# YichengDWu/tinyedm

Measured on AMD Instinct MI355X. Metric: train imgs/sec CIFAR-10 32x32 bf16, higher is better.
Workload: dtype bf16; 1 GPU; CIFAR-10 32x32 unconditional EDM2 U-Net (conf/cifar10.yaml, 35.6M params) full training step: diffuse+embed+denoiser fwd/bwd+loss+grad all-reduce+Adam+EMA; per_gpu_batch=128, global_batch=128, parallelism=dp1, conditional=False, step_launch=hipGraph replay, collective=none

## Files before the change

include/tinyedm_hip.h:

```cpp
#ifndef TINYEDM_HIP_H
#define TINYEDM_HIP_H
#ifdef __cplusplus
extern "C" {
#endif

typedef struct ihipStream_t* edm_stream_t;

int edm_version(void);
const char* edm_last_error(void);
int edm_init(int device);
int edm_graph_replay_safe(void);
typedef struct {
  unsigned step, seed_lo, seed_hi, reserved;
  float lr, ema_beta, grad_scale, bc1, bc2sqrt, pad[3];
} edm_step_params;

int edm_conv_igemm(const void* X, const void* Wp, void* Y, const void* R, float alpha, float beta, int B, int H,
                   int W, int Cin, int Cout, int taps, edm_stream_t stream);
int edm_conv_igemm_v2(const void* X, const void* Wp, void* Y, const void* R, float alpha, float beta, int B, int H,
                      int W, int Cin, int Cout, int taps, edm_stream_t stream);
int edm_conv_igemm_v6(const void* X, const void* Wp, void* Y, const void* R, float alpha, float beta, int B, int H,
                      int W, int Cin, int Cout, int taps, edm_stream_t stream);
int edm_conv_igemm_s(const void* X, const void* Wp, void* Y, const void* R, float alpha, float beta, int B, int H,
                     int W, int Cin, int Cout, int taps, edm_stream_t stream);
// ... 82 lines not shown
int edm_attention_fwd(const void* qkv, void* y, int B, int N, int C, int heads, edm_stream_t stream);
int edm_attention_bwd(const void* qkv, const void* y, const void* gy, void* gqkv, int B, int N, int C, int heads,
                      edm_stream_t stream);

int edm_attention_long_supported(int N, int C, int heads);
int edm_attention_long_fwd(const void* qkv, void* y, float* stat, int B, int N, int C, int heads, edm_stream_t stream);
int edm_attention_long_bwd(const void* qkv, const void* y, const void* gy, const float* stat, void* gqkv, float* work,
                           int B, int N, int C, int heads, edm_stream_t stream);

int edm_attention_qkv_supported(int N, int C, int heads);
int edm_attention_qkv_fwd(const void* x, const void* Wqkv, void* y, void* stat, int B, int N, int C, int heads,
                          int heads_per_wg, edm_stream_t stream);
int edm_attention_qkv_bwd(const void* x, const void* y, const void* gout, const void* stat, const void* Wqkv,
                          const void* Wd_out, void* gqkv, float alpha, int B, int N, int C, int heads, int heads_per_wg,
                          edm_stream_t stream);

int edm_pixelnorm_silu_fwd(const void* x, void* xn, void* a, float* dsave, long P, int C, edm_stream_t stream);
int edm_pixelnorm_silu_bwd(const void* xn, const float* dsave, const void* gxn, float gxn_scale, const void* ga,
                           const void* gadd, void* gx, long P, int C, edm_stream_t stream);
int edm_pool_pixelnorm_silu_fwd(const void* x, void* xn, void* a, float* dsave, int B, int Hp, int Wp, int C,
                                edm_stream_t stream);
int edm_pool_pixelnorm_silu_bwd(const void* xn, const float* dsave, const void* gxn, float gxn_scale, const void* ga,
                                const void* gadd, void* gx, int B, int Hp, int Wp, int C, edm_stream_t stream);
int edm_silu_fwd(const void* x, void* a, long n, edm_stream_t stream);
int edm_silu_bwd(const void* x, const void* ga, const void* gextra, float extra_scale, void* gx, long n,
                 edm_stream_t stream);
int edm_axpby(const void* a, float alpha, const void* b, float beta, void* out, long n, edm_stream_t stream);
int edm_mod_silu_drop_fwd(const void* r, const float* lin, long lin_stride, const float* gain, void* a, int B, int HW,
                          int C, float pdrop, unsigned long long seed, unsigned sub, unsigned step, const void* dyn,
                          edm_stream_t stream);
int edm_mod_silu_drop_bwd(const void* r, const float* lin, long lin_stride, const float* gain, const void* ga, void* gr,
                          float* gm, float* glin, long glin_stride, float* ggain, int B, int HW, int C, float pdrop,
                          unsigned long long seed, unsigned sub, unsigned step, const void* dyn, edm_stream_t stream);
int edm_mod_silu_drop_bwd_raw(const void* r, const float* lin, long lin_stride, const float* gain, const void* ga, void* gr,
                              float* gm, long gm_stride, int B, int HW, int C, float pdrop, unsigned long long seed,
                              unsigned sub, unsigned step, const void* dyn, edm_stream_t stream);
int edm_dropout_mask(unsigned char* mask, long n, float pdrop, unsigned long long seed, unsigned sub, unsigned step,
                     edm_stream_t stream);
int edm_pool2(const void* x, void* y, int B, int Hout, int Wout, int C, float scale, edm_stream_t stream);
int edm_up2(const void* x, const void* add, void* y, int B, int Hout, int Wout, int C, float scale, edm_stream_t stream);
int edm_up2_silu(const void* x, void* y, void* a, int B, int Hout, int Wout, int C, edm_stream_t stream);
int edm_reduce_hw(const void* x, long x_stride, const void* y, long y_stride, float* out, int B, int HW, int C,
                  float scale, edm_stream_t stream);
int edm_scalelong_fwd(const float* mean, const float* W1h, const float* W2h, float* gate, float* z1save, int B, int C,
                      int R, edm_stream_t stream);
int edm_scalelong_bwd(const float* mean, const float* W1h, const float* W2h, const float* gate, const float* z1save,
// ... 278 lines not shown
```

tinyedm_amd/_lib.py:

```python
import ctypes
import os

_HERE = os.path.dirname(os.path.abspath(__file__))
LIB_PATH = os.environ.get("EDM_LIB_PATH") or os.path.join(_HERE, "libtinyedm_hip.so")

P, I, L, F = ctypes.c_void_p, ctypes.c_int, ctypes.c_long, ctypes.c_float
U, U64 = ctypes.c_uint, ctypes.c_ulonglong
D = ctypes.c_double

SIGNATURES = {
    "edm_version": [],
    "edm_last_error": [],
    "edm_init": [I],
    "edm_graph_replay_safe": [],
    "edm_pixelnorm_silu_fwd": [P, P, P, P, L, I, P],
    "edm_pixelnorm_silu_bwd": [P, P, P, F, P, P, P, L, I, P],
    "edm_pool_pixelnorm_silu_fwd": [P, P, P, P, I, I, I, I, P],
    "edm_pool_pixelnorm_silu_bwd": [P, P, P, F, P, P, P, I, I, I, I, P],
    "edm_up2_silu": [P, P, P, I, I, I, I, P],
    "edm_silu_fwd": [P, P, L, P],
    "edm_silu_bwd": [P, P, P, F, P, L, P],
    "edm_axpby": [P, F, P, F, P, L, P],
    "edm_mod_silu_drop_fwd": [P, P, L, P, P, I, I, I, F, U64, U, U, P, P],
    "edm_mod_silu_drop_bwd": [P, P, L, P, P, P, P, P, L, P, I, I, I, F, U64, U, U, P, P],
    "edm_mod_silu_drop_bwd_raw": [P, P, L, P, P, P, P, L, I, I, I, F, U64, U, U, P, P],
    "edm_dropout_mask": [P, L, F, U64, U, U, P],
    "edm_pool2": [P, P, I, I, I, I, F, P],
    "edm_up2": [P, P, P, I, I, I, I, F, P],
    "edm_reduce_hw": [P, L, P, L, P, I, I, I, F, P],
    "edm_scalelong_fwd": [P, P, P, P, P, I, I, I, P],
    "edm_scalelong_bwd": [P, P, P, P, P, P, P, P, P, I, I, I, P],
    "edm_skip_gate_fwd": [P, P, P, P, P, P, I, I, I, I, P],
    "edm_skip_gate_bwd": [P, L, I, P, P, P, P, P, P, P, P, P, P, I, I, I, I, P],
    "edm_skip_gate_wgrad_multi": [P, I, P, P, I, P],
    "edm_skip_gate_wgrad_multi_table_bytes": [],
    "edm_skip_gate_fwd_multi": [P, I, P, P, I, P],
    "edm_skip_gate_fwd_multi_table_bytes": [],
    "edm_skip_gate_bwd_multi": [P, I, P, P, I, P],
    "edm_skip_half_bwd_multi": [P, I, P, P, I, P],
    "edm_skip_gate_bwd_multi_table_bytes": [],
    "edm_concat_gate_fwd": [P, P, P, P, P, I, I, I, I, P],
# ... 243 lines not shown
```

tinyedm_amd/csrc/elementwise.hip:

```cpp
#include "common.h"
#include <stdarg.h>
#include <stdio.h>

static thread_local char g_err[512] = "";
extern "C" void edm_set_error(const char* fmt, ...) {
  va_list ap;
  va_start(ap, fmt);
  vsnprintf(g_err, sizeof(g_err), fmt, ap);
  va_end(ap);
}
extern "C" const char* edm_last_error() { return g_err; }
extern "C" int edm_version() { return 1; }

static inline int cdiv(long a, long b) { return (int)((a + b - 1) / b); }
static inline int grid_for(long work, int block, int cap = 256 * 16) {
  long g = (work + block - 1) / block;
  if (g > cap) g = cap;
  if (g < 1) g = 1;
  return (int)g;
}

template <int LPP, bool POOL = false>
__global__ __launch_bounds__(256) void k_pnorm_silu_fwd(const bf16* __restrict__ x, bf16* __restrict__ xn,
                                                          bf16* __restrict__ a, float* __restrict__ dsave, int P,
// ... 35 lines not shown
      }
    }
    ss = group_sum<LPP>(ss);
    const float d = NORM_EPS + sqrtf(ss) * rsC;
    const float inv = 1.0f / d;
#pragma unroll
    for (int it = 0; it < 2; ++it) {
      const int c8 = lig + it * LPP;
      if (pv && c8 < CL) {
        float o[8], s[8];
#pragma unroll
        for (int i = 0; i < 8; ++i) {
          o[i] = (float)(bf16)(v[it][i] * inv);
          s[i] = mp_silu_b(o[i]);
        }
        store8(xn + p * C + c8 * 8, o);
        store8(a + p * C + c8 * 8, s);
      }
    }
    if (pv && lig == 0) dsave[p] = d;
  }
}

template <int LPP, bool UP = false>
__global__ __launch_bounds__(256) void k_pnorm_silu_bwd(const bf16* __restrict__ xn, const float* __restrict__ dsave,
                                                          const bf16* __restrict__ gxn, float gs,
                                                          const bf16* __restrict__ ga, const bf16* __restrict__ gadd,
                                                          bf16* __restrict__ gx, int P, int C, int Hp = 0, int Wp = 0) {
  constexpr int GPW = 64 / LPP;
  const int lane = threadIdx.x & 63, wave = threadIdx.x >> 6;
  const int lig = lane % LPP, grp = lane / LPP;
  const int CL = C >> 3;
  const long stride = (long)gridDim.x * 4 * GPW;
  for (long p0 = ((long)blockIdx.x * 4 + wave) * GPW; p0 < P; p0 += stride) {
    const long p = p0 + grp;
    const bool pv = p < P;
    float y[2][8], g[2][8];
    float dot = 0.f;
#pragma unroll
    for (int it = 0; it < 2; ++it) {
      const int c8 = lig + it * LPP;
      if (pv && c8 < CL) {
        load8(xn + p * C + c8 * 8, y[it]);
        float t[8];
        if (gxn) {
          load8(gxn + p * C + c8 * 8, t);
#pragma unroll
          for (int i = 0; i < 8; ++i) g[it][i] = gs * t[i];
        } else {
#pragma unroll
          for (int i = 0; i < 8; ++i) g[it][i] = 0.f;
// ... 14 lines not shown
    float inv = 1.0f / d;
#pragma unroll
    for (int it = 0; it < 2; ++it) {
      const int c8 = lig + it * LPP;
      if (pv && c8 < CL) {
        float o[8];
#pragma unroll
        for (int i = 0; i < 8; ++i) o[i] = (g[it][i] - y[it][i] * coef) * inv;
        if constexpr (UP) {
          const int w = (int)(p % Wp);
          const long t2 = p / Wp;
          const int h = (int)(t2 % Hp);
          const long b = t2 / Hp;
          const long e0 = ((b * 2 * Hp + 2 * h) * 2 * Wp + 2 * w) * C + c8 * 8;
          const long row = (long)2 * Wp * C;
#pragma unroll
          for (int i = 0; i < 8; ++i) o[i] = 0.25f * (float)(bf16)o[i];
#pragma unroll
          for (int q = 0; q < 4; ++q) {
            const long e = e0 + (q >> 1) * row + (q & 1) * C;
            float r[8];
#pragma unroll
            for (int i = 0; i < 8; ++i) r[i] = o[i];
            if (gadd) {
              float t[8];
              load8(gadd + e, t);
#pragma unroll
              for (int i = 0; i < 8; ++i) r[i] += t[i];
            }
            store8(gx + e, r);
          }
          continue;
        }
        if (gadd) {
          float t[8];
          load8(gadd + p * C + c8 * 8, t);
#pragma unroll
          for (int i = 0; i < 8; ++i) o[i] += t[i];
        }
        store8(gx + p * C + c8 * 8, o);
      }
    }
  }
}

static int pick_lpp(int C) {
  int cl = C / 8;
  return cl <= 16 ? 16 : (cl <= 32 ? 32 : 64);
}

extern "C" int edm_pixelnorm_silu_fwd(const void* x, void* xn, void* a, float* dsave, long P, int C,
                                      hipStream_t st) {
  EDM_REQUIRE(P > 0 && P < (1L << 31) && C > 0 && C % 8 == 0 && C <= 1024, "pixelnorm_silu_fwd: bad P=%ld C=%d", P, C);
  int lpp = pick_lpp(C);
  int gpw = 64 / lpp;
  int grid = grid_for(P, 4 * gpw);
#define L(N) hipLaunchKernelGGL(k_pnorm_silu_fwd<N>, dim3(grid), dim3(256), 0, st, (const bf16*)x, (bf16*)xn, (bf16*)a, dsave, (int)P, C)
// ... 23 lines not shown
  EDM_REQUIRE(xn && dsave && gx && B > 0 && Hp > 0 && Wp > 0 && C > 0 && C % 8 == 0 && C <= 1024 &&
                  (long)B * Hp * Wp < (1L << 31), "pool_pixelnorm_silu_bwd: bad args");
  const long P = (long)B * Hp * Wp;
  int lpp = pick_lpp(C);
  int gpw = 64 / lpp;
  int grid = grid_for(P, 4 * gpw);
#define L(N) hipLaunchKernelGGL((k_pnorm_silu_bwd<N, true>), dim3(grid), dim3(256), 0, st, (const bf16*)xn, dsave, (const bf16*)gxn, gxn_scale, (const bf16*)ga, (const bf16*)gadd, (bf16*)gx, (int)P, C, Hp, Wp)
  if (lpp == 16) L(16); else if (lpp == 32) L(32); else L(64);
#undef L
  EDM_CHECK_LAUNCH("pool_pixelnorm_silu_bwd");
  return EDM_OK;
}

extern "C" int edm_pixelnorm_silu_bwd(const void* xn, const float* dsave, const void* gxn, float gxn_scale,
                                      const void* ga, const void* gadd, void* gx, long P, int C, hipStream_t st) {
  EDM_REQUIRE(P > 0 && P < (1L << 31) && C > 0 && C % 8 == 0 && C <= 1024, "pixelnorm_silu_bwd: bad P=%ld C=%d", P, C);
  int lpp = pick_lpp(C);
  int gpw = 64 / lpp;
  int grid = grid_for(P, 4 * gpw);
#define L(N) hipLaunchKernelGGL(k_pnorm_silu_bwd<N>, dim3(grid), dim3(256), 0, st, (const bf16*)xn, dsave, (const bf16*)gxn, gxn_scale, (const bf16*)ga, (const bf16*)gadd, (bf16*)gx, (int)P, C)
  if (lpp == 16) L(16); else if (lpp == 32) L(32); else L(64);
#undef L
  EDM_CHECK_LAUNCH("pixelnorm_silu_bwd");
  return EDM_OK;
}

__global__ void k_silu_fwd(const bf16* __restrict__ x, bf16* __restrict__ a, long n8) {
  for (long i = (long)blockIdx.x * blockDim.x + threadIdx.x; i < n8; i += (long)gridDim.x * blockDim.x) {
    float v[8];
    load8(x + i * 8, v);
#pragma unroll
    for (int j = 0; j < 8; ++j) v[j] = mp_silu_b(v[j]);
    store8(a + i * 8, v);
  }
}
__global__ void k_silu_bwd(const bf16* __restrict__ x, const bf16* __restrict__ ga, const bf16* __restrict__ ge,
                           float s, bf16* __restrict__ gx, long n8) {
  for (long i = (long)blockIdx.x * blockDim.x + threadIdx.x; i < n8; i += (long)gridDim.x * blockDim.x) {
    float v[8], g[8], e[8];
    load8(x + i * 8, v);
    load8(ga + i * 8, g);
    if (ge) load8(ge + i * 8, e);
#pragma unroll
    for (int j = 0; j < 8; ++j) g[j] = mp_silu_grad_b(v[j]) * g[j] + (ge ? s * e[j] : 0.f);
    store8(gx + i * 8, g);
  }
// ... 1358 lines not shown
```

tinyedm_amd/networks.py:

```python
from __future__ import annotations

import contextlib
import math
import os
from typing import Optional

import numpy as np
import torch
import torch.nn as nn
from torch import Tensor

from . import ops

bf16, f32 = torch.bfloat16, torch.float32


class _Rng:
    seed: int = 42
    step: int = 0
    dyn = None


rng = _Rng()

# ... 82 lines not shown
                _flush_fin(key)
            _queue_backward_end(w.device)
            return None
        g = ops.wgrad_finish(slabs, w.data, self._taps(), I, perm=self._perm, scale=scale)
        return g.view_as(w)


WGRAD_STREAM = os.environ.get("EDM_WGRAD_STREAM", "1") != "0"
W3_GROUP = max(0, min(ops.W3_MAX_LAYERS, int(os.environ.get("EDM_W3_GROUP", "16"))))
W3_TAIL = max(0, int(os.environ.get("EDM_W3_TAIL", "0")))
_w3_seen = {}
_w3_total = {}
W3_MAXPIX = int(os.environ.get("EDM_W3_MAXPIX", str(1 << 18)))
FIN_GROUP = 40
W1_GROUP = max(0, min(16, int(os.environ.get("EDM_W1_GROUP", "16"))))
_w1_pending = {}
_bwd_end_queued = set()
MOD_DEFER_UNFUSED = os.environ.get("EDM_MOD_DEFER_UNFUSED", "1") != "0"
SG_MULTI = os.environ.get("EDM_SG_MULTI", "1") != "0"
SG_HALVES = os.environ.get("EDM_SG_HALVES", "1") != "0"
SG_BWD_MULTI = os.environ.get("EDM_SG_BWD_MULTI", "1") != "0"
SG_DEFER = os.environ.get("EDM_SG_DEFER", "1") != "0"
_sg_pending = {}
_w3_pending = {}
TAIL_LOWRANK = os.environ.get("EDM_TAIL_LOWRANK", "1") != "0"
_tail_slot = {}
TAIL_FWD = os.environ.get("EDM_TAIL_FWD", "1") != "0"
_tail_fwd_slot = {}
_fin_pending = {}


def _run_on_side(device, fn, tensors=()):
    if WGRAD_STREAM:
        side = ops.side_stream(device)
        side.wait_stream(torch.cuda.current_stream())
        with torch.cuda.stream(side):
            fn()
        for t in tensors:
            t.record_stream(side)
    else:
        fn()


class FusedOptPass:

    def __init__(self, base, ema, dyn):
# ... 64 lines not shown
    _run_on_side(dev, lambda: ops.wgrad_finish_multi(args), [a[0] for a in args])
    for _, w, *_rest in items:
        w._edm_deferred = False
        for hook in getattr(w, "_edm_hooks", ()):
            hook(w)


def _flush_sg(key):
    items = _sg_pending.pop(key, None)
    if not items:
        return
    outs = ops.skip_gate_wgrad_multi([(ws, mean, R) for _, ws, mean, R in items])
    for (sl, _, _, _), (gw1h, gw2h) in zip(items, outs):
        sl.layer1.finish_grad(gw1h.view(1, 1, *gw1h.shape))
        sl.layer2.finish_grad(gw2h.view(1, 1, *gw2h.shape))


def _backward_end(key):
    _bwd_end_queued.discard(key)
    _tail_slot.pop(key, None)
    _tail_fwd_slot.pop(key, None)
    if key in _w3_seen:
        _w3_total[key] = _w3_seen.pop(key)
    _flush_sg(key)
    _flush_w3(key)
    _flush_fin(key)
    if WGRAD_STREAM:
        torch.cuda.current_stream(key).wait_stream(ops.side_stream(key))


def _queue_backward_end(device):
    key = torch.device(device).index
    if key in _bwd_end_queued:
        return
    try:
        torch.autograd.Variable._execution_engine.queue_callback(lambda: _backward_end(key))
        _bwd_end_queued.add(key)
    except RuntimeError:
        _backward_end(key)


def reset_backward_state():
    _tail_slot.clear()
    _tail_fwd_slot.clear()
    if _bwd_end_queued or _w3_pending or _fin_pending or _w1_pending or _sg_pending:
        _bwd_end_queued.clear()
        for items in _sg_pending.values():
            for sl, *_rest in items:
                sl.layer1.weight._edm_deferred = sl.layer2.weight._edm_deferred = False
        _sg_pending.clear()
        for items in _w1_pending.values():
            for m, _, _, _ in items:
                m.weight._edm_deferred = False
        _w1_pending.clear()
        for items in _fin_pending.values():
            for _, w, *_rest in items:
                w._edm_deferred = False
        _fin_pending.clear()
        for items in _w3_pending.values():
            for m, _, _, _ in items:
                m.weight._edm_deferred = False
        _w3_pending.clear()
        _w3_seen.clear()
        if WGRAD_STREAM:
            for s in ops.side_streams():
                torch.cuda.current_stream(s.device).wait_stream(s)

# ... 611 lines not shown
        gw_qkv = _wgrad(mod.qkv_conv, x, gqkv, 1)
        return gx, gw_qkv, gw_out, None, None, None


class _ResBlockFn(torch.autograd.Function):

    @staticmethod
    def forward(ctx, u, emb, w1x1, w1, w2, wemb, gain, blk, lin_view, glin_view, token, s_pre=None, alias=False,
                gm_view=None, skip=None, w_sl1=None, w_sl2=None, pre=None, dest=None, pool=False, gate_pre=None, tail=0):
        enc = blk.is_encoder
        ctx.set_materialize_grads(False)
        has1 = w1x1 is not None
        taps = 9
        wf1, wd1, _ = blk.conv_3x3_1.packs()
        wf2, wd2, _ = blk.conv_3x3_2.packs()
        batched = lin_view is not None
        weh = None if batched else blk.embed.packs()[2]
        wf11 = wd11 = None
        tail_fwd = False
        ctx.has_skip = skip is not None
        if skip is not None:
            sl = blk.cat_factor
            ctx.sgb = None
            if gate_pre is not None:
                mean, gate, z1, w1h, w2h, ctx.sgb, halves = gate_pre
            else:
                w1h, w2h = sl.layer1.packs()[2], sl.layer2.packs()[2]
                mean, gate, z1 = ops.skip_gate_fwd(skip, w1h, w2h)
            ctx.Ci = u.shape[-1]
            if pre is not None and pre[0].shape[-1] == u.shape[-1] + skip.shape[-1] and pre[0].data_ptr() == u.data_ptr():
                cat, s_pre = pre
                if not (gate_pre is not None and halves == cat.data_ptr()):
                    ops.skip_half_fwd(skip, gate, cat, s_pre)
            else:
                cat, s_pre = ops.concat_gate_fwd(u.contiguous(), skip, gate, True)
            u = cat
            ctx.skip_saved = (skip, mean, gate, z1, w1h, w2h)
        ctx.pool = bool(pool)
        if enc and pool:
            assert not has1
            xres, s, dsave = ops.pool_pixelnorm_silu_fwd(u)
        elif enc:
            x = u
            if has1:
                wf11, wd11, _ = blk.conv_1x1.packs()
                x = ops.conv_igemm(u, wf11, 1)
            xres, s, dsave = ops.pixelnorm_silu_fwd(x)
        else:
# ... 28 lines not shown
                out = ops.conv3x3_fold(a2, wf2, u, wf11, b, a, out=_col_block(dest[0], Co), silu_out=_col_block(dest[1], Co))
                out._edm_cat = dest
            else:
                out = ops.conv3x3_fold(a2, wf2, u, wf11, b, a)
        elif _dest_ok(dest, a2):
            out = ops.conv_igemm(a2, wf2, taps, residual=xres, alpha=b, beta=a, out=_col_block(dest[0], Co),
                                 silu_out=_col_block(dest[1], Co))
            out._edm_cat = dest
        else:
            out = ops.conv_igemm(a2, wf2, taps, residual=xres, alpha=b, beta=a)
        ctx.blk, ctx.enc, ctx.has1 = blk, enc, has1
        ctx.tail_fwd = tail_fwd
        ctx.drop = (pdrop, seed, sub, step, rng.dyn)
        ctx.u_marked = U_MARKS and ops.FUSE_MOD and ops.IGEMM_VERSION == 0
        ctx.batched, ctx.glin_view, ctx.gm_view = batched, glin_view, gm_view
        ctx.has_token = token is not None
        ctx.save_for_backward(u if (not enc or has1) else None, xres if enc else None, dsave, s, r1, lin, a2,
                              None if batched else emb, gain, wd1, wd2, wd11, weh)
        return (out, u) if alias else out

    @staticmethod
    def backward(ctx, gout, g_alias=None):
        u, xn, dsave, s, r1, lin, a2, emb, gain, wd1, wd2, wd11, weh = ctx.saved_tensors
        if g_alias is not None:
            g_alias = g_alias.contiguous()
        blk, enc, has1 = ctx.blk, ctx.enc, ctx.has1
        pdrop, seed, sub, step, dyn = ctx.drop
        gout = gout.contiguous()
        a, b = _mp_coeffs(blk.add_factor)
        glin_out = ctx.glin_view if ctx.batched else None
        gp = blk.gain
        gdirect = gp.grad is not None and getattr(gp, "_edm_direct", False) and gp.grad.is_contiguous()
        ggain_out = gp.grad if gdirect else None
        deferred = False
        fused = ops.FUSE_MOD and ops.IGEMM_VERSION == 0 and (gout.shape[1] * gout.shape[2]) % 32 == 0
        only = _DGRAD_ONLY[0]
        gm_only = ops.zeros_f32((lin.shape[0], lin.shape[-1]), gout.device) if only else None

        def gm_of(deferred):
            return gm_only if only else (ctx.gm_view if deferred else None)
        tail = tfwd = None
        if ctx.tail_fwd:
            slot = _tail_slot.pop(gout.device.index, None)
            if slot is None or len(slot) != 7 or r1 is None:
                raise RuntimeError("tinyedm_amd: the last block's backward ran without the output end's (TAIL_FWD: its "
                                   "output is a handle that only _TailOutFn consumes)")
            tail, tfwd = slot[:2], slot[3:]
        elif blk._tail_last:
            slot = _tail_slot.pop(gout.device.index, None)
# ... 76 lines not shown
                    ops.conv_igemm(gout, wd11, 1, residual=t, alpha=a, beta=1.0, split=(Ci, gu, gcs))
                else:
                    gu = ops.conv_igemm(gout, wd11, 1, residual=t, alpha=a, beta=1.0)
                    gcs = None
                gw11 = _wgrad(blk.conv_1x1, u, gout, 1, a)
            else:
                gu = ops.conv3x3_silubwd(gr1, wd1, u, gout, a) if fuse else ops.silu_bwd(u, gs, gout, a)
                gcs = None
        gskip = gwsl1 = gwsl2 = None
        if ctx.has_skip:
            skip, mean, gate, z1, w1h, w2h = ctx.skip_saved
            Ci = ctx.Ci
            sl = blk.cat_factor
            wsl = (sl.layer1.weight, sl.layer2.weight)
            defer = SG_DEFER and all(w.grad is not None and getattr(w, "_edm_direct", False) for w in wsl)
            sgb = getattr(ctx, "sgb", None)
            queued = False
            if only:
                if gcs is None:
                    gmean, _ws = ops.skip_gate_bwd(gu, Ci, skip, mean, w1h, w2h, gate, z1, defer_wgrad=True)
                    gu, gskip = ops.concat_gate_bwd(gu, gate, gmean, Ci)
                elif defer and sgb is not None and SG_BWD_MULTI:
                    gskip = torch.empty_like(gcs)
                    sgb.pending.append((gcs, skip, w1h, w2h, gate, z1, gskip, sl, mean))
                else:
                    gmean, _ws = ops.skip_gate_bwd(gcs, 0, skip, mean, w1h, w2h, gate, z1, defer_wgrad=True)
                    gskip = ops.skip_half_bwd(gcs, gate, gmean)
            elif gcs is None:
                gmean, *gws = ops.skip_gate_bwd(gu, Ci, skip, mean, w1h, w2h, gate, z1, defer_wgrad=defer)
                gu, gskip = ops.concat_gate_bwd(gu, gate, gmean, Ci)
            elif defer and sgb is not None and SG_BWD_MULTI:
                gskip = torch.empty_like(gcs)
                sgb.pending.append((gcs, skip, w1h, w2h, gate, z1, gskip, sl, mean))
                queued = True
            else:
                gmean, *gws = ops.skip_gate_bwd(gcs, 0, skip, mean, w1h, w2h, gate, z1, defer_wgrad=defer)
                gskip = ops.skip_half_bwd(gcs, gate, gmean)
            if only:
                pass
            elif defer:
                if not queued:
                    _sg_pending.setdefault(wsl[0].device.index, []).append((sl, gws[0], mean, w1h.shape[0]))
                wsl[0]._edm_deferred = wsl[1]._edm_deferred = True
                _queue_backward_end(wsl[0].device)
            else:
                gw1h, gw2h = gws
                gwsl1 = sl.layer1.finish_grad(gw1h.view(1, 1, *gw1h.shape))
                gwsl2 = sl.layer2.finish_grad(gw2h.view(1, 1, *gw2h.shape))
            if sgb is not None:
                sgb.arrived += 1
                if sgb.arrived == sgb.expected:
                    sgb.flush()
        if g_alias is not None:
            gu = ops.axpby(gu, 1.0, g_alias, 1.0)
        return (gu, gemb, gw11, gw1, gw2, gwemb, ggain, None, None, None, gtoken, None, None, None, gskip, gwsl1, gwsl2,
                None, None, None, None, None)
# ... 109 lines not shown


def _tag(x: Tensor) -> Tensor:
    x._edm_nhwc = True
    return x


class EncoderBlock(_BlockBase):
    is_encoder = True

    def __init__(self, in_channels: int, out_channels: int, embedding_dim: int, down: bool, attention: bool,
                 num_heads: int = 4, dropout_rate: float = 0.0, add_factor: float = 0.3):
        super().__init__()
        self.dropout_rate = dropout_rate
        self.add_factor = add_factor
        self.resample = DownSample() if down else nn.Identity()
        self.conv_1x1 = Conv2d(in_channels, out_channels, 1) if in_channels != out_channels else nn.Identity()
        self.conv_3x3_1 = Conv2d(out_channels, out_channels, 3)
        self._common(out_channels, embedding_dim, attention, num_heads, dropout_rate)

    def forward(self, input: Tensor, embedding: Tensor, _lin=None, _alias: bool = False, _dest=None):
        x, conv = _as_nhwc(input)
        ualias = None
        emb = None if _lin is not None else _emb32(embedding, x.shape[0])
        if (isinstance(self.resample, DownSample) and FUSE_RESAMPLE and not isinstance(self.conv_1x1, Conv2d)
                and x.shape[-1] <= 1024 and x.shape[1] % 2 == 0 and x.shape[2] % 2 == 0):
            out = self._res(x, emb, _lin, alias=_alias, pool=True, dest=_dest)
            if _alias:
                out, ualias = out
        else:
            if isinstance(self.resample, DownSample):
                if _alias:
                    x, ualias = _ResampleFn.apply(x, False, True)
                else:
                    x = _ResampleFn.apply(x, False)
            if _alias and ualias is None:
                out, ualias = self._res(x, emb, _lin, alias=True, dest=_dest)
            else:
                out = self._res(x, emb, _lin, dest=_dest)
        if conv:
            out = ops.nhwc_bf16_to_nchw(out).to(input.dtype)
        else:
            cat_pre = getattr(out, "_edm_cat", None)
            out = _tag(out)
            if cat_pre is not None:
                out._edm_cat = cat_pre
        return (out, _tag(ualias)) if _alias else out

    def forward_f32(self, x: Tensor, lin: Tensor, want=None):
        pairs = _split_ok(self.conv_3x3_1)
        if (F32_FUSE_OUT and isinstance(self.resample, DownSample) and not isinstance(self.conv_1x1, Conv2d)
                and x.shape[-1] <= 1024):
            xn, s = ops.f32_pool_pixelnorm_silu(x, pairs=pairs)
        else:
            if isinstance(self.resample, DownSample):
                x = ops.f32_pool2(x)
            if isinstance(self.conv_1x1, Conv2d):
                x = _conv_f32(self.conv_1x1, x, 1)
            xn, s = ops.f32_pixelnorm_silu(x, pairs=pairs)
        return _res_f32(self, xn, s, lin, want)


class DecoderBlock(_BlockBase):
    is_encoder = False

    def __init__(self, in_channels: int, out_channels: int, embedding_dim: int, up: bool, attention: bool,
                 num_heads: int = 4, skip_channels: int = 0, dropout_rate: float = 0.0, add_factor: float = 0.3):
        super().__init__()
        self.add_factor = add_factor
        self.dropout_rate = dropout_rate
# ... 631 lines not shown
        D = self._conv_out_of(x, noisy, sig, link)
        if self.training:
            rng.step += 1
        return D.to(noisy_image.dtype)


class _SgbPass:

    def __init__(self, expected: int):
        self.expected, self.arrived, self.pending = expected, 0, []

    def flush(self):
        items, self.pending = self.pending, []
        self.arrived = 0
        if not items:
            return
        by_c = {}
        for it in items:
            by_c.setdefault(it[1].shape[-1], []).append(it)
        halves = []
        for group in by_c.values():
            for k0 in range(0, len(group), 32):
                part = group[k0:k0 + 32]
                res = ops.skip_gate_bwd_multi([(gcs, 0, skip, w1h, w2h, gate, z1) + ((gskip,) if SG_HALVES else ())
                                               for gcs, skip, w1h, w2h, gate, z1, gskip, _, _ in part])
                for (gcs, skip, w1h, w2h, gate, z1, gskip, sl, mean), (gmean, ws) in zip(part, res):
                    if not SG_HALVES:
                        halves.append((gcs, gate, gmean, gskip))
                    if _DGRAD_ONLY[0]:
                        continue
                    _sg_pending.setdefault(sl.layer1.weight.device.index, []).append((sl, ws, mean, w1h.shape[0]))
        for k0 in range(0, len(halves), 32):
            ops.skip_half_bwd_multi(halves[k0:k0 + 32])


def _decoder_dests_impl(dec, skips, x):
    out = {}
    st = list(skips)
    h, w = x.shape[1], x.shape[2]
    for i, (block, has_skip) in enumerate(dec):
        if has_skip:
            st.pop()
        if isinstance(block.resample, UpSample):
            h, w = 2 * h, 2 * w
        if i + 1 < len(dec) and dec[i + 1][1]:
            nxt = dec[i + 1][0]
            if not isinstance(nxt.resample, UpSample) and isinstance(nxt.conv_1x1, Conv2d):
                Ct = block.conv_3x3_2.weight.shape[0] + st[-1].shape[-1]
                out[i] = (torch.empty(x.shape[0], h, w, Ct, device=x.device, dtype=bf16),
                          torch.empty(x.shape[0], h, w, Ct, device=x.device, dtype=bf16))
    return out


def _decoder_gates_impl(dec, skips, dests=None):
    st = list(skips)
    todo = {}
    for i, (block, has_skip) in enumerate(dec):
        if not has_skip:
            continue
        skip = st.pop()
        if not (isinstance(block, DecoderBlock) and block._gate_in_block() and skip.dim() == 4 and skip.dtype == bf16):
            continue
        sl = block.cat_factor
        pre = dests.get(i - 1) if dests and SG_HALVES else None
        if pre is not None and not (pre[0].shape[:3] == skip.shape[:3] and pre[0].shape[-1] > skip.shape[-1]):
            pre = None
        todo.setdefault(skip.shape[-1], []).append((block, skip, sl.layer1.packs()[2], sl.layer2.packs()[2], pre))
    out = {}
    tok = _SgbPass(sum(len(v) for v in todo.values())) if torch.is_grad_enabled() else None
    for items in todo.values():
        for k0 in range(0, len(items), 32):
            part = items[k0:k0 + 32]
            res = ops.skip_gate_fwd_multi([(skip, w1h, w2h) + (pre if pre is not None else ()) for _, skip, w1h, w2h, pre in part])
            for (block, _, w1h, w2h, pre), (mean, gate, z1) in zip(part, res):
                out[block] = (mean, gate, z1, w1h, w2h, tok, None if pre is None else pre[0].data_ptr())
    return out


class DenoiserWrapper(nn.Module):

    def __init__(self, net: nn.Module, sigma_data: float):
        super().__init__()
        self.net = net
        self._sigma_data = sigma_data

    @property
    def sigma_data(self) -> float:
        return self._sigma_data

    def forward(self, noisy_image: Tensor, sigma: Tensor, embedding: Tensor | None = None) -> Tensor:
        sigma = sigma.view(-1, 1, 1, 1)
        sd = self.sigma_data
        c_skip = sd ** 2 / (sigma ** 2 + sd ** 2)
        c_out = sigma * sd / (sigma ** 2 + sd ** 2).sqrt()
        c_in = 1 / (sd ** 2 + sigma ** 2).sqrt()
        c_noise = sigma.log() / 4
        F_ = self.net(c_in * noisy_image, c_noise.flatten(), embedding)
        return c_skip * noisy_image + c_out * F_
# ... 1 lines not shown
```

tinyedm_amd/ops.py:

```python
import contextlib
import ctypes
import functools
import math
import os
import types
from typing import Optional

import torch

from . import _lib

bf16, f32 = torch.bfloat16, torch.float32

PROFILE = None


class _prof:
    def __init__(self, name, flops, nbytes):
        self.name, self.flops, self.nbytes = name, flops, nbytes

    def __enter__(self):
        if PROFILE is not None:
            self.s = torch.cuda.Event(enable_timing=True)
            self.e = torch.cuda.Event(enable_timing=True)
            self.s.record()
        return self

    def __exit__(self, *a):
        if PROFILE is not None:
# ... 263 lines not shown
        raise TypeError(f"{name}: expected {dtype}, got {t.dtype}")
    if not t.is_contiguous():
        raise ValueError(f"{name}: must be contiguous")
    if shape is not None and tuple(t.shape) != tuple(shape):
        raise ValueError(f"{name}: expected shape {tuple(shape)}, got {tuple(t.shape)}")
    return t


def _nhwc(t, name):
    _chk(t, bf16, name)
    if t.dim() != 4:
        raise ValueError(f"{name}: expected (B,H,W,C)")
    return t.shape


def pixelnorm_silu_fwd(x):
    B, H, W, C = _nhwc(x, "x")
    xn, a = torch.empty_like(x), torch.empty_like(x)
    d = torch.empty(B * H * W, device=x.device, dtype=f32)
    _lib.call("edm_pixelnorm_silu_fwd", _p(x), _p(xn), _p(a), _p(d), B * H * W, C, _stream())
    return xn, a, d


def pixelnorm_silu_bwd(xn, d, gxn, gxn_scale, ga, gadd=None):
    B, H, W, C = _nhwc(xn, "xn")
    _chk(d, f32, "d", (B * H * W,))
    if gxn is not None:
        _chk(gxn, bf16, "gxn", xn.shape)
    if ga is not None:
        _chk(ga, bf16, "ga", xn.shape)
    if gadd is not None:
        _chk(gadd, bf16, "gadd", xn.shape)
    gx = torch.empty_like(xn)
    _lib.call("edm_pixelnorm_silu_bwd", _p(xn), _p(d), _p(gxn), float(gxn_scale), _p(ga), _p(gadd), _p(gx), B * H * W, C,
              _stream())
    return gx


def pool_pixelnorm_silu_fwd(x):
    B, H, W, C = _nhwc(x, "x")
    if H % 2 or W % 2 or C > 1024:
        raise ValueError("pool_pixelnorm_silu_fwd: H, W even and C <= 1024 required")
    xn = torch.empty(B, H // 2, W // 2, C, device=x.device, dtype=bf16)
    a = torch.empty_like(xn)
    d = torch.empty(B * (H // 2) * (W // 2), device=x.device, dtype=f32)
    _lib.call("edm_pool_pixelnorm_silu_fwd", _p(x), _p(xn), _p(a), _p(d), B, H // 2, W // 2, C, _stream())
    return xn, a, d


def pool_pixelnorm_silu_bwd(xn, d, gxn, gxn_scale, ga, gadd=None):
    B, H, W, C = _nhwc(xn, "xn")
    _chk(d, f32, "d", (B * H * W,))
    if gxn is not None:
        _chk(gxn, bf16, "gxn", xn.shape)
    if ga is not None:
        _chk(ga, bf16, "ga", xn.shape)
    if gadd is not None:
        _chk(gadd, bf16, "gadd", (B, 2 * H, 2 * W, C))
    gx = torch.empty(B, 2 * H, 2 * W, C, device=xn.device, dtype=bf16)
    _lib.call("edm_pool_pixelnorm_silu_bwd", _p(xn), _p(d), _p(gxn), float(gxn_scale), _p(ga), _p(gadd), _p(gx), B, H, W, C,
              _stream())
    return gx


def up2_silu(x):
    B, H, W, C = _nhwc(x, "x")
    y = torch.empty(B, 2 * H, 2 * W, C, device=x.device, dtype=bf16)
    a = torch.empty_like(y)
    _lib.call("edm_up2_silu", _p(x), _p(y), _p(a), B, 2 * H, 2 * W, C, _stream())
    return y, a


def silu_fwd(x):
    _chk(x, bf16, "x")
    a = torch.empty_like(x)
    _lib.call("edm_silu_fwd", _p(x), _p(a), x.numel(), _stream())
    return a


# ... 2552 lines not shown
```

Before: 10790 img/s.

## Defer skip-gradient materialisation and fuse it into pixelnorm-SiLU backward

```diff
diff --git a/include/tinyedm_hip.h b/include/tinyedm_hip.h
--- a/include/tinyedm_hip.h
+++ b/include/tinyedm_hip.h
@@ -128,6 +128,12 @@
                                 edm_stream_t stream);
 int edm_pool_pixelnorm_silu_bwd(const void* xn, const float* dsave, const void* gxn, float gxn_scale, const void* ga,
                                 const void* gadd, void* gx, int B, int Hp, int Wp, int C, edm_stream_t stream);
+int edm_pixelnorm_silu_bwd_lazy(const void* xn, const float* dsave, const void* gxn, float gxn_scale, const void* ga,
+                                const void* gcat, long gcat_stride, int c_off, const float* gate, const float* gmean, int HW,
+                                void* gx, long P, int C, edm_stream_t stream);
+int edm_pool_pixelnorm_silu_bwd_lazy(const void* xn, const float* dsave, const void* gxn, float gxn_scale, const void* ga,
+                                     const void* gcat, long gcat_stride, int c_off, const float* gate, const float* gmean,
+                                     void* gx, int B, int Hp, int Wp, int C, edm_stream_t stream);
 int edm_silu_fwd(const void* x, void* a, long n, edm_stream_t stream);
 int edm_silu_bwd(const void* x, const void* ga, const void* gextra, float extra_scale, void* gx, long n,
                  edm_stream_t stream);
diff --git a/tinyedm_amd/_lib.py b/tinyedm_amd/_lib.py
--- a/tinyedm_amd/_lib.py
+++ b/tinyedm_amd/_lib.py
@@ -17,6 +17,8 @@
     "edm_pixelnorm_silu_bwd": [P, P, P, F, P, P, P, L, I, P],
     "edm_pool_pixelnorm_silu_fwd": [P, P, P, P, I, I, I, I, P],
     "edm_pool_pixelnorm_silu_bwd": [P, P, P, F, P, P, P, I, I, I, I, P],
+    "edm_pixelnorm_silu_bwd_lazy": [P, P, P, F, P, P, L, I, P, P, I, P, L, I, P],
+    "edm_pool_pixelnorm_silu_bwd_lazy": [P, P, P, F, P, P, L, I, P, P, P, I, I, I, I, P],
     "edm_up2_silu": [P, P, P, I, I, I, I, P],
     "edm_silu_fwd": [P, P, L, P],
     "edm_silu_bwd": [P, P, P, F, P, L, P],
diff --git a/tinyedm_amd/csrc/elementwise.hip b/tinyedm_amd/csrc/elementwise.hip
--- a/tinyedm_amd/csrc/elementwise.hip
+++ b/tinyedm_amd/csrc/elementwise.hip
@@ -81,11 +81,27 @@
   }
 }
 
-template <int LPP, bool UP = false>
+struct LazyGadd {
+  const bf16* gcat;
+  const float* gate;
+  const float* gmean;
+  long gs;
+  float inv_hw;
+  int HW;
+};
+__device__ __forceinline__ void lazy_gadd8(const LazyGadd& lz, long pix, long b, int cs, int C, float (&t)[8]) {
+  load8(lz.gcat + pix * lz.gs + cs, t);
+  const float* gp = lz.gate + b * C + cs;
+  const float* mp = lz.gmean + b * C + cs;
+#pragma unroll
+  for (int j = 0; j < 8; ++j) t[j] = (float)(bf16)(t[j] * gp[j] + mp[j] * lz.inv_hw);
+}
+template <int LPP, bool UP = false, bool LAZY = false>
 __global__ __launch_bounds__(256) void k_pnorm_silu_bwd(const bf16* __restrict__ xn, const float* __restrict__ dsave,
                                                           const bf16* __restrict__ gxn, float gs,
                                                           const bf16* __restrict__ ga, const bf16* __restrict__ gadd,
-                                                          bf16* __restrict__ gx, int P, int C, int Hp = 0, int Wp = 0) {
+                                                          bf16* __restrict__ gx, int P, int C, int Hp = 0, int Wp = 0,
+                                                          LazyGadd lz = LazyGadd{}) {
   constexpr int GPW = 64 / LPP;
   const int lane = threadIdx.x & 63, wave = threadIdx.x >> 6;
   const int lig = lane % LPP, grp = lane / LPP;
@@ -146,7 +162,15 @@
             float r[8];
 #pragma unroll
             for (int i = 0; i < 8; ++i) r[i] = o[i];
-            if (gadd) {
+            if constexpr (LAZY) {
+              float t[8];
+              lazy_gadd8(lz, ((b * 2 * Hp + 2 * h + (q >> 1)) * 2 * Wp + 2 * w + (q & 1)), b, c8 * 8, C, t);
+#pragma unroll
+              for (int i = 0; i < 8; ++i) {
+                asm volatile("" : "+v"(r[i]));
+                r[i] += t[i];
+              }
+            } else if (gadd) {
               float t[8];
               load8(gadd + e, t);
 #pragma unroll
@@ -156,7 +180,15 @@
           }
           continue;
         }
-        if (gadd) {
+        if constexpr (LAZY) {
+          float t[8];
+          lazy_gadd8(lz, p, p / lz.HW, c8 * 8, C, t);
+#pragma unroll
+          for (int i = 0; i < 8; ++i) {
+            asm volatile("" : "+v"(o[i]));
+            o[i] += t[i];
+          }
+        } else if (gadd) {
           float t[8];
           load8(gadd + p * C + c8 * 8, t);
 #pragma unroll
@@ -226,6 +258,49 @@
   if (lpp == 16) L(16); else if (lpp == 32) L(32); else L(64);
 #undef L
   EDM_CHECK_LAUNCH("pixelnorm_silu_bwd");
+  return EDM_OK;
+}
+
+static int lazy_gadd_args(const char* who, const void* gcat, long gcat_stride, int c_off, const float* gate,
+                          const float* gmean, int C) {
+  EDM_REQUIRE(gcat && gate && gmean && c_off >= 0 && c_off % 8 == 0 && gcat_stride % 8 == 0 && gcat_stride >= (long)c_off + C,
+              "%s: bad lazy skip-gradient descriptor", who);
+  return EDM_OK;
+}
+extern "C" int edm_pixelnorm_silu_bwd_lazy(const void* xn, const float* dsave, const void* gxn, float gxn_scale,
+                                           const void* ga, const void* gcat, long gcat_stride, int c_off,
+                                           const float* gate, const float* gmean, int HW, void* gx, long P, int C,
+                                           hipStream_t st) {
+  EDM_REQUIRE(xn && dsave && gx && P > 0 && P < (1L << 31) && C > 0 && C % 8 == 0 && C <= 1024 && HW > 0 && P % HW == 0,
+              "pixelnorm_silu_bwd_lazy: bad P=%ld C=%d HW=%d", P, C, HW);
+  if (int rc = lazy_gadd_args("pixelnorm_silu_bwd_lazy", gcat, gcat_stride, c_off, gate, gmean, C)) return rc;
+  const LazyGadd lz{(const bf16*)gcat + c_off, gate, gmean, gcat_stride, 1.0f / (float)HW, HW};
+  int lpp = pick_lpp(C);
+  int gpw = 64 / lpp;
+  int grid = grid_for(P, 4 * gpw);
+#define L(N) hipLaunchKernelGGL((k_pnorm_silu_bwd<N, false, true>), dim3(grid), dim3(256), 0, st, (const bf16*)xn, dsave, (const bf16*)gxn, gxn_scale, (const bf16*)ga, (const bf16*)nullptr, (bf16*)gx, (int)P, C, 0, 0, lz)
+  if (lpp == 16) L(16); else if (lpp == 32) L(32); else L(64);
+#undef L
+  EDM_CHECK_LAUNCH("pixelnorm_silu_bwd_lazy");
+  return EDM_OK;
+}
+extern "C" int edm_pool_pixelnorm_silu_bwd_lazy(const void* xn, const float* dsave, const void* gxn, float gxn_scale,
+                                                const void* ga, const void* gcat, long gcat_stride, int c_off,
+                                                const float* gate, const float* gmean, void* gx, int B, int Hp, int Wp,
+                                                int C, hipStream_t st) {
+  EDM_REQUIRE(xn && dsave && gx && B > 0 && Hp > 0 && Wp > 0 && C > 0 && C % 8 == 0 && C <= 1024 &&
+                  (long)B * Hp * Wp < (1L << 29), "pool_pixelnorm_silu_bwd_lazy: bad args");
+  if (int rc = lazy_gadd_args("pool_pixelnorm_silu_bwd_lazy", gcat, gcat_stride, c_off, gate, gmean, C)) return rc;
+  const long P = (long)B * Hp * Wp;
+  const int HW = 4 * Hp * Wp;
+  const LazyGadd lz{(const bf16*)gcat + c_off, gate, gmean, gcat_stride, 1.0f / (float)HW, HW};
+  int lpp = pick_lpp(C);
+  int gpw = 64 / lpp;
+  int grid = grid_for(P, 4 * gpw);
+#define L(N) hipLaunchKernelGGL((k_pnorm_silu_bwd<N, true, true>), dim3(grid), dim3(256), 0, st, (const bf16*)xn, dsave, (const bf16*)gxn, gxn_scale, (const bf16*)ga, (const bf16*)nullptr, (bf16*)gx, (int)P, C, Hp, Wp, lz)
+  if (lpp == 16) L(16); else if (lpp == 32) L(32); else L(64);
+#undef L
+  EDM_CHECK_LAUNCH("pool_pixelnorm_silu_bwd_lazy");
   return EDM_OK;
 }
 
diff --git a/tinyedm_amd/networks.py b/tinyedm_amd/networks.py
--- a/tinyedm_amd/networks.py
+++ b/tinyedm_amd/networks.py
@@ -128,6 +128,37 @@
 SG_BWD_MULTI = os.environ.get("EDM_SG_BWD_MULTI", "1") != "0"
 SG_DEFER = os.environ.get("EDM_SG_DEFER", "1") != "0"
 _sg_pending = {}
+SG_LAZY = os.environ.get("EDM_SG_LAZY", "1") != "0"
+_sg_lazy = {}
+
+
+def _take_lazy(g: Tensor, usable: bool):
+    slot = _sg_lazy.get(g.device.index)
+    if not slot:
+        return None
+    entry = slot.get(g.data_ptr())
+    if entry is None or entry[0].shape != g.shape or not g.is_contiguous():
+        return None
+    del slot[g.data_ptr()]
+    if usable:
+        return entry[1]
+    _materialise_lazy([entry])
+    return None
+
+
+def _materialise_lazy(entries):
+    for k0 in range(0, len(entries), 32):
+        ops.skip_half_bwd_multi([(lz.gcat, lz.gate, lz.gmean, ph) for ph, lz in entries[k0:k0 + 32]])
+
+
+def _flush_lazy(key):
+    slot = _sg_lazy.pop(key, None)
+    if slot:
+        _materialise_lazy(list(slot.values()))
+
+
+def _skip_observed(skip: Tensor) -> bool:
+    return bool(skip.retains_grad or getattr(skip, "_backward_hooks", None) or getattr(skip, "_post_accumulate_grad_hooks", None))
 _w3_pending = {}
 TAIL_LOWRANK = os.environ.get("EDM_TAIL_LOWRANK", "1") != "0"
 _tail_slot = {}
@@ -238,6 +269,7 @@
     _tail_fwd_slot.pop(key, None)
     if key in _w3_seen:
         _w3_total[key] = _w3_seen.pop(key)
+    _flush_lazy(key)
     _flush_sg(key)
     _flush_w3(key)
     _flush_fin(key)
@@ -259,6 +291,7 @@
 def reset_backward_state():
     _tail_slot.clear()
     _tail_fwd_slot.clear()
+    _sg_lazy.clear()
     if _bwd_end_queued or _w3_pending or _fin_pending or _w1_pending or _sg_pending:
         _bwd_end_queued.clear()
         for items in _sg_pending.values():
@@ -916,8 +949,9 @@
         if skip is not None:
             sl = blk.cat_factor
             ctx.sgb = None
+            ctx.lazy_ok = False
             if gate_pre is not None:
-                mean, gate, z1, w1h, w2h, ctx.sgb, halves = gate_pre
+                mean, gate, z1, w1h, w2h, ctx.sgb, halves, ctx.lazy_ok = gate_pre
             else:
                 w1h, w2h = sl.layer1.packs()[2], sl.layer2.packs()[2]
                 mean, gate, z1 = ops.skip_gate_fwd(skip, w1h, w2h)
@@ -992,9 +1026,10 @@
     @staticmethod
     def backward(ctx, gout, g_alias=None):
         u, xn, dsave, s, r1, lin, a2, emb, gain, wd1, wd2, wd11, weh = ctx.saved_tensors
+        blk, enc, has1 = ctx.blk, ctx.enc, ctx.has1
         if g_alias is not None:
-            g_alias = g_alias.contiguous()
-        blk, enc, has1 = ctx.blk, ctx.enc, ctx.has1
+            lazy = _take_lazy(g_alias, enc and (ctx.pool or not has1)) if _sg_lazy else None
+            g_alias = lazy if lazy is not None else g_alias.contiguous()
         pdrop, seed, sub, step, dyn = ctx.drop
         gout = gout.contiguous()
         a, b = _mp_coeffs(blk.add_factor)
@@ -1117,7 +1152,7 @@
                     gu, gskip = ops.concat_gate_bwd(gu, gate, gmean, Ci)
                 elif defer and sgb is not None and SG_BWD_MULTI:
                     gskip = torch.empty_like(gcs)
-                    sgb.pending.append((gcs, skip, w1h, w2h, gate, z1, gskip, sl, mean))
+                    sgb.pending.append((gcs, skip, w1h, w2h, gate, z1, gskip, sl, mean, False))
                 else:
                     gmean, _ws = ops.skip_gate_bwd(gcs, 0, skip, mean, w1h, w2h, gate, z1, defer_wgrad=True)
                     gskip = ops.skip_half_bwd(gcs, gate, gmean)
@@ -1126,7 +1161,8 @@
                 gu, gskip = ops.concat_gate_bwd(gu, gate, gmean, Ci)
             elif defer and sgb is not None and SG_BWD_MULTI:
                 gskip = torch.empty_like(gcs)
-                sgb.pending.append((gcs, skip, w1h, w2h, gate, z1, gskip, sl, mean))
+                lazy = SG_LAZY and ctx.lazy_ok and gcs.is_contiguous() and not _skip_observed(skip)
+                sgb.pending.append((gcs, skip, w1h, w2h, gate, z1, gskip, sl, mean, lazy))
                 queued = True
             else:
                 gmean, *gws = ops.skip_gate_bwd(gcs, 0, skip, mean, w1h, w2h, gate, z1, defer_wgrad=defer)
@@ -1282,12 +1318,14 @@
     def forward(self, input: Tensor, embedding: Tensor, _lin=None, _alias: bool = False, _dest=None):
         x, conv = _as_nhwc(input)
         ualias = None
+        lazy_ok = False
         emb = None if _lin is not None else _emb32(embedding, x.shape[0])
         if (isinstance(self.resample, DownSample) and FUSE_RESAMPLE and not isinstance(self.conv_1x1, Conv2d)
                 and x.shape[-1] <= 1024 and x.shape[1] % 2 == 0 and x.shape[2] % 2 == 0):
             out = self._res(x, emb, _lin, alias=_alias, pool=True, dest=_dest)
             if _alias:
                 out, ualias = out
+                lazy_ok = True
         else:
             if isinstance(self.resample, DownSample):
                 if _alias:
@@ -1296,6 +1334,7 @@
                     x = _ResampleFn.apply(x, False)
             if _alias and ualias is None:
                 out, ualias = self._res(x, emb, _lin, alias=True, dest=_dest)
+                lazy_ok = not isinstance(self.conv_1x1, Conv2d) and x.shape[-1] <= 1024
             else:
                 out = self._res(x, emb, _lin, dest=_dest)
         if conv:
@@ -1305,7 +1344,11 @@
             out = _tag(out)
             if cat_pre is not None:
                 out._edm_cat = cat_pre
-        return (out, _tag(ualias)) if _alias else out
+        if _alias:
+            ualias = _tag(ualias)
+            ualias._edm_lazy_ok = lazy_ok and not (self._backward_hooks or self._backward_pre_hooks)
+            return out, ualias
+        return out
 
     def forward_f32(self, x: Tensor, lin: Tensor, want=None):
         pairs = _split_ok(self.conv_3x3_1)
@@ -1983,10 +2026,12 @@
         for group in by_c.values():
             for k0 in range(0, len(group), 32):
                 part = group[k0:k0 + 32]
-                res = ops.skip_gate_bwd_multi([(gcs, 0, skip, w1h, w2h, gate, z1) + ((gskip,) if SG_HALVES else ())
-                                               for gcs, skip, w1h, w2h, gate, z1, gskip, _, _ in part])
-                for (gcs, skip, w1h, w2h, gate, z1, gskip, sl, mean), (gmean, ws) in zip(part, res):
-                    if not SG_HALVES:
+                res = ops.skip_gate_bwd_multi([(gcs, 0, skip, w1h, w2h, gate, z1) + ((gskip,) if SG_HALVES and not lazy else ())
+                                               for gcs, skip, w1h, w2h, gate, z1, gskip, _, _, lazy in part])
+                for (gcs, skip, w1h, w2h, gate, z1, gskip, sl, mean, lazy), (gmean, ws) in zip(part, res):
+                    if lazy:
+                        _sg_lazy.setdefault(gskip.device.index, {})[gskip.data_ptr()] = (gskip, ops.LazySkipGrad(gcs, 0, gate, gmean))
+                    elif not SG_HALVES:
                         halves.append((gcs, gate, gmean, gskip))
                     if _DGRAD_ONLY[0]:
                         continue
@@ -2033,8 +2078,9 @@
         for k0 in range(0, len(items), 32):
             part = items[k0:k0 + 32]
             res = ops.skip_gate_fwd_multi([(skip, w1h, w2h) + (pre if pre is not None else ()) for _, skip, w1h, w2h, pre in part])
-            for (block, _, w1h, w2h, pre), (mean, gate, z1) in zip(part, res):
-                out[block] = (mean, gate, z1, w1h, w2h, tok, None if pre is None else pre[0].data_ptr())
+            for (block, skip, w1h, w2h, pre), (mean, gate, z1) in zip(part, res):
+                out[block] = (mean, gate, z1, w1h, w2h, tok, None if pre is None else pre[0].data_ptr(),
+                              getattr(skip, "_edm_lazy_ok", False))
     return out
 
 
diff --git a/tinyedm_amd/ops.py b/tinyedm_amd/ops.py
--- a/tinyedm_amd/ops.py
+++ b/tinyedm_amd/ops.py
@@ -4,7 +4,7 @@
 import math
 import os
 import types
-from typing import Optional
+from typing import NamedTuple, Optional
 
 import torch
 
@@ -314,6 +314,24 @@
     return xn, a, d
 
 
+class LazySkipGrad(NamedTuple):
+    gcat: torch.Tensor
+    c_off: int
+    gate: torch.Tensor
+    gmean: torch.Tensor
+
+
+def _chk_lazy(lz, shape):
+    B, H, W, C = shape
+    Ct = lz.gcat.shape[-1] if lz.gcat.dim() == 4 else 0
+    _chk(lz.gcat, bf16, "gadd.gcat", (B, H, W, Ct))
+    if lz.c_off < 0 or lz.c_off % 8 or Ct % 8 or lz.c_off + C > Ct:
+        raise ValueError("gadd: columns [c_off, c_off + C) must lie inside gcat, c_off and gcat's width multiples of 8")
+    _chk(lz.gate, f32, "gadd.gate", (B, C))
+    _chk(lz.gmean, f32, "gadd.gmean", (B, C))
+    return Ct
+
+
 def pixelnorm_silu_bwd(xn, d, gxn, gxn_scale, ga, gadd=None):
     B, H, W, C = _nhwc(xn, "xn")
     _chk(d, f32, "d", (B * H * W,))
@@ -321,6 +339,12 @@
         _chk(gxn, bf16, "gxn", xn.shape)
     if ga is not None:
         _chk(ga, bf16, "ga", xn.shape)
+    if isinstance(gadd, LazySkipGrad):
+        Ct = _chk_lazy(gadd, xn.shape)
+        gx = torch.empty_like(xn)
+        _lib.call("edm_pixelnorm_silu_bwd_lazy", _p(xn), _p(d), _p(gxn), float(gxn_scale), _p(ga), _p(gadd.gcat), Ct,
+                  int(gadd.c_off), _p(gadd.gate), _p(gadd.gmean), H * W, _p(gx), B * H * W, C, _stream())
+        return gx
     if gadd is not None:
         _chk(gadd, bf16, "gadd", xn.shape)
     gx = torch.empty_like(xn)
@@ -347,6 +371,12 @@
         _chk(gxn, bf16, "gxn", xn.shape)
     if ga is not None:
         _chk(ga, bf16, "ga", xn.shape)
+    if isinstance(gadd, LazySkipGrad):
+        Ct = _chk_lazy(gadd, (B, 2 * H, 2 * W, C))
+        gx = torch.empty(B, 2 * H, 2 * W, C, device=xn.device, dtype=bf16)
+        _lib.call("edm_pool_pixelnorm_silu_bwd_lazy", _p(xn), _p(d), _p(gxn), float(gxn_scale), _p(ga), _p(gadd.gcat), Ct,
+                  int(gadd.c_off), _p(gadd.gate), _p(gadd.gmean), _p(gx), B, H, W, C, _stream())
+        return gx
     if gadd is not None:
         _chk(gadd, bf16, "gadd", (B, 2 * H, 2 * W, C))
     gx = torch.empty(B, 2 * H, 2 * W, C, device=xn.device, dtype=bf16)
```

Result: no change. 10860 img/s (median of 6 runs) (+0.7%).
